# robotic-vision-lab/CropNeRF-A-Neural-Radiance-Field-Based-Framework

Hardware: NVIDIA B200
Metric: train_rays_per_s (higher is better)
Workload: dtype f16 tensor-core MLPs (bf16 gradients), f32 hash tables / accumulation / compositing

## Files before the change

### cropnerf-a-neural-radiance-field-based-framework_b200/csrc/field_mixed_bwd.cu

```cuda
#include <cstdlib>

#include "field_mixed.cuh"

using namespace cnbmix;

namespace {

constexpr int ST = 72;
constexpr int BATCH = WARPS * 16;
constexpr int T_R3 = 0;
constexpr int T_R2 = T_R3 + 64 * 24;
constexpr int T_R1 = T_R2 + 64 * 72;
constexpr int T_S2 = T_R1 + 64 * 72;
constexpr int T_B2 = T_S2 + 64 * 72;
constexpr int T_B1 = T_B2 + 64 * 24;
constexpr int T_HALVES = T_B1 + 32 * 72;
constexpr int A_R3 = 0, A_R2 = 1, A_R1 = 5, A_H = 9, A_S2 = 10, A_S1 = 14, A_B2 = 15, A_B1 = 16, A_TILES = 18;
constexpr int B_R3 = 0, B_R2 = 16, B_R1 = 80, B_H = 144, B_S2 = 160, B_S1 = 224, B_B2 = 288, B_B1 = 304, B_FLOATS = 368;

constexpr size_t SMEM_BWD = (size_t)(HALVES + T_HALVES + 4 * BATCH * ST) * 2 + (size_t)(FLOATS + B_FLOATS + WARPS * A_TILES * 128) * 4;
constexpr int SC_WARPS = 4;
constexpr int THREADS_FUSED = THREADS + SC_WARPS * 32;
constexpr int NSLOT = 4;
constexpr size_t SMEM_BWD_FUSED = SMEM_BWD + 2 * NSLOT * sizeof(uint64_t);
static_assert(BATCH == SC_WARPS * 32, "one scatter warp per 32 samples of a batch");
static_assert(SMEM_BWD_FUSED <= 232448, "227 KB of dynamic shared memory per CTA");

struct BwdArgs {
  MixArgs m;
  float* d_table;
  const __half* x0;
  const float* pos;
  const float *d_density, *d_rgb, *d_sem;
  float* d_x0;
  float *dWb1, *dbb1, *dWb2, *dbb2, *dWs1, *dbs1, *dWs2, *dbs2, *dWh, *dbh, *dWr1, *dbr1, *dWr2, *dbr2, *dWr3, *dbr3;
  float* d_embedding;
};

__device__ __forceinline__ uint32_t pack_bf2(float a, float b) {
  __nv_bfloat162 h = __floats2bfloat162_rn(a, b);
  return *reinterpret_cast<uint32_t*>(&h);
}
__device__ __forceinline__ float2 unpack_h2(uint32_t v) { return __half22float2(*reinterpret_cast<__half2*>(&v)); }
__device__ __forceinline__ uint32_t h2_to_bf2(uint32_t v) {
  const float2 f = unpack_h2(v);
// ... 97 lines not shown
__device__ __forceinline__ void flush_tiles(const float* acc_tiles, int warp, int lane, Put put) {
  constexpr int WPM = WARPS / MT;
  constexpr int NT = NTT / WPM;
  const int mi = warp / WPM, nj0 = (warp % WPM) * NT;
  const int g = lane >> 2, t = lane & 3;
#pragma unroll
  for (int nt = 0; nt < NT; ++nt)
#pragma unroll
    for (int q = 0; q < 4; ++q) {
      const float v = acc_tiles[(nt * 4 + q) * 32 + lane];
      if (v != 0.f) put(16 * mi + g + (q >> 1) * 8, 8 * (nj0 + nt) + 2 * t + (q & 1), v);
    }
}

__device__ __forceinline__ void bar_mlp() { asm volatile("bar.sync 1, %0;" ::"n"(THREADS) : "memory"); }
__device__ __forceinline__ void mbar_arrive(uint32_t bar) { asm volatile("mbarrier.arrive.shared::cta.b64 _, [%0];" ::"r"(bar) : "memory"); }
__device__ __forceinline__ void mbar_wait(uint32_t bar, uint32_t parity) {
  uint32_t done;
  do {
    asm volatile("{\n\t.reg .pred p;\n\tmbarrier.try_wait.parity.shared::cta.b64 p, [%1], %2;\n\tselp.b32 %0, 1, 0, p;\n\t}" : "=r"(done) : "r"(bar), "r"(parity) : "memory");
  } while (!done);
}

__device__ __forceinline__ void scatter_role(const MixArgs& a, float* __restrict__ d_table, const float* __restrict__ pos, const float* __restrict__ d_x0,
                                             uint32_t mbar_s, int sw, int lane, int64_t N, int64_t nbatches) {
  int j = 0;
  for (int64_t batch = blockIdx.x; batch < nbatches; batch += gridDim.x, ++j) {
    const int slot = j % NSLOT;
    const uint32_t par = (uint32_t)(j / NSLOT) & 1u;
    const int64_t s = batch * BATCH + sw * 32 + lane;
    const bool in = s < N;
    float px = 0.f, py = 0.f, pz = 0.f;
    if (in) { px = __ldg(pos + 3 * s); py = __ldg(pos + 3 * s + 1); pz = __ldg(pos + 3 * s + 2); }
    mbar_wait(mbar_s + 8 * slot, par);
#pragma unroll 1
    for (int l0 = 0; l0 < a.L; l0 += 4) {
      float2 d[4];
#pragma unroll
      for (int q = 0; q < 4; ++q) {
        d[q] = make_float2(0.f, 0.f);
        if (in && l0 + q < a.L) d[q] = __ldcg(reinterpret_cast<const float2*>(d_x0) + (int64_t)(l0 + q) * N + s);
      }
#pragma unroll
      for (int q = 0; q < 4; ++q) {
        const int l = l0 + q;
        if (l < a.L) {
          const bool active = d[q].x != 0.0f || d[q].y != 0.0f;
          CnbCell c = {};
          if (active) c = cnb_cell(px, py, pz, a.scalings[l]);
          cnb_scatter_cell(d_table, c, a.mask, (uint32_t)l * a.T, d[q].x, d[q].y, active);
        }
      }
    }
    __syncwarp();
    if (lane == 0) mbar_arrive(mbar_s + 8 * (NSLOT + slot));
  }
}

__device__ inline void load_weights_t(const MixArgs& a, __nv_bfloat16* WT) {
  const int tid = threadIdx.x;
  for (int e = tid; e < 64 * 24; e += THREADS) {
    const int in = e / 24, out = e - in * 24;
    WT[T_R3 + e] = __float2bfloat16_rn(out < 3 ? __ldg(a.Wr3 + out * 64 + in) : 0.f);
    WT[T_B2 + e] = __float2bfloat16_rn(out < 16 ? __ldg(a.Wb2 + out * 64 + in) : 0.f);
  }
  for (int e = tid; e < 64 * 72; e += THREADS) {
    const int in = e / 72, out = e - in * 72;
    const bool ok = out < 64;
    WT[T_R2 + e] = __float2bfloat16_rn(ok ? __ldg(a.Wr2 + out * 64 + in) : 0.f);
    WT[T_S2 + e] = __float2bfloat16_rn(ok ? __ldg(a.Ws2 + out * 64 + in) : 0.f);
    float w1 = 0.f;
    if (ok) {
      if (in < 16) w1 = __ldg(a.Wr1 + out * 63 + in);
      else if (in >= 17) w1 = __ldg(a.Wr1 + out * 63 + (in - 1));
    }
    WT[T_R1 + e] = __float2bfloat16_rn(w1);
  }
  for (int e = tid; e < 32 * 72; e += THREADS) {
    const int in = e / 72, out = e - in * 72;
    WT[T_B1 + e] = __float2bfloat16_rn((out < 64 && in < a.in0) ? __ldg(a.Wb1 + out * a.in0 + in) : 0.f);
  }
}

template <bool FUSED>
__global__ void __launch_bounds__(FUSED ? THREADS_FUSED : THREADS, 1) k_field_mixed_bwd(const __grid_constant__ BwdArgs b) {
  extern __shared__ __align__(16) unsigned char smem_raw[];
  const MixArgs& a = b.m;
  __half* Wsm = reinterpret_cast<__half*>(smem_raw);
  __nv_bfloat16* WT = reinterpret_cast<__nv_bfloat16*>(Wsm + HALVES);
  __nv_bfloat16* st_base = WT + T_HALVES;
  float* Bf = reinterpret_cast<float*>(st_base + 4 * BATCH * ST);
  float* bias_acc = Bf + FLOATS;
  float* acc_all = bias_acc + B_FLOATS;
  const uint32_t mbar_s = (uint32_t)__cvta_generic_to_shared(smem_raw + SMEM_BWD);
  if (!FUSED || threadIdx.x < THREADS) {
    load_weights(a, Wsm, Bf);
    load_weights_t(a, WT);
    for (int e = threadIdx.x; e < B_FLOATS + WARPS * A_TILES * 128; e += THREADS) bias_acc[e] = 0.f;
  } else if (threadIdx.x == THREADS) {
    for (int i = 0; i < NSLOT; ++i) {
      asm volatile("mbarrier.init.shared::cta.b64 [%0], %1;" ::"r"(mbar_s + 8 * i), "r"(THREADS));
      asm volatile("mbarrier.init.shared::cta.b64 [%0], %1;" ::"r"(mbar_s + 8 * (NSLOT + i)), "r"(SC_WARPS));
    }
    asm volatile("fence.mbarrier_init.release.cluster;" ::: "memory");
  }
  __syncthreads();

  const int warp = threadIdx.x >> 5, lane = threadIdx.x & 31;
  if (FUSED) {
    const int64_t N_ = a.sm.num_rays * a.sm.samples_per_ray;
    if (warp >= WARPS) {
      asm volatile("setmaxnreg.dec.sync.aligned.u32 56;");
      scatter_role(a, b.d_table, b.pos, b.d_x0, mbar_s, warp - WARPS, lane, N_, (N_ + BATCH - 1) / BATCH);
      return;
    }
    asm volatile("setmaxnreg.inc.sync.aligned.u32 224;");
  }
  const int g = lane >> 2, t = lane & 3;
  float* acc_w = acc_all + warp * A_TILES * 128;
  uint32_t* const st32 = reinterpret_cast<uint32_t*>(st_base);
  const uint32_t st_s = (uint32_t)__cvta_generic_to_shared(st_base);
  constexpr int MATW = BATCH * ST / 2;
  int buf = 0;
  const int row0 = warp * 16;
  const int S = a.sm.samples_per_ray;
  const int64_t N = a.sm.num_rays * S;
  const int64_t nbatches = (N + BATCH - 1) / BATCH;

  struct TileIn {
    uint32_t A0[2][4];
    float dirv[2][3];
    float2 embv[2][2][2];
// ... 38 lines not shown
        if (t == 0 && b.d_density) { in.ddens[h] = __ldg(b.d_density + rw); in.posx[h] = __ldg(b.pos + 3 * rw); }
      }
    }
  };
  const int64_t tstride = (int64_t)gridDim.x * WARPS;
  TileIn nxt;
  int cam2[2];
  {
    const int64_t t0 = (int64_t)blockIdx.x * WARPS + warp;
    int cam1[2];
    load_cam(t0, cam1);
    load_tile(t0, cam1, nxt);
    load_cam(t0 + tstride, cam2);
  }

  int jb = 0;
  for (int64_t batch = blockIdx.x; batch < nbatches; batch += gridDim.x, ++jb) {
    const int64_t tile = batch * WARPS + warp;
    const int64_t row[2] = {tile * 16 + g, tile * 16 + g + 8};
    bool valid[2];
#pragma unroll
    for (int h = 0; h < 2; ++h) valid[h] = row[h] < N;
    const TileIn cur = nxt;
    load_tile(tile + tstride, cam2, nxt);
    load_cam(tile + 2 * tstride, cam2);
    uint32_t A0[2][4];
#pragma unroll
    for (int kt = 0; kt < 2; ++kt)
#pragma unroll
      for (int q = 0; q < 4; ++q) A0[kt][q] = cur.A0[kt][q];
    const int cam[2] = {cur.cam[0], cur.cam[1]};
    const float (&dirv)[2][3] = cur.dirv;
// ... 177 lines not shown
      uint32_t D[4][4];
      relu_mask_pack<4>(acc, AH, D);
      stage<4, false>(st32 + (2 * buf + 1) * MATW, row0, D, g, t);
      stage<2, true>(st32 + (2 * buf) * MATW, row0, A0, g, t);
      bar_mlp();
      dw_gemm<4, 4>(st_s + (2 * buf + 1) * MATW * 4, st_s + (2 * buf) * MATW * 4, acc_w + A_B1 * 128, bias_acc + B_B1, warp, lane);
      buf ^= 1;
      float dx[4][4];
      zero_acc<4>(dx);
      layer_bf<4, 4, 72>(WT + T_B1, D, dx, g, t);
#pragma unroll
      for (int nt = 0; nt < 4; ++nt) {
        float2* const dlev = reinterpret_cast<float2*>(b.d_x0) + (int64_t)(4 * nt + t) * N;
        if (valid[0]) dlev[row[0]] = make_float2(dx[nt][0], dx[nt][1]);
        if (valid[1]) dlev[row[1]] = make_float2(dx[nt][2], dx[nt][3]);
      }
      if (FUSED) {
        const int slot = jb % NSLOT;
        if (jb >= NSLOT) mbar_wait(mbar_s + 8 * (NSLOT + slot), (uint32_t)(jb / NSLOT - 1) & 1u);
        mbar_arrive(mbar_s + 8 * slot);
      }
    }
  }

  const int in0 = a.in0;
  if (b.dWr3) flush_tiles<1, 8>(acc_w + A_R3 * 128, warp, lane, [&](int n, int k, float v) { if (n < 3) atomicAdd(b.dWr3 + n * 64 + k, v); });
  if (b.dWr2) flush_tiles<4, 8>(acc_w + A_R2 * 128, warp, lane, [&](int n, int k, float v) { atomicAdd(b.dWr2 + n * 64 + k, v); });
  if (b.dWr1) flush_tiles<4, 8>(acc_w + A_R1 * 128, warp, lane, [&](int n, int k, float v) { if (k != 16) atomicAdd(b.dWr1 + n * 63 + (k < 16 ? k : k - 1), v); });
  if (b.dWh) flush_tiles<1, 8>(acc_w + A_H * 128, warp, lane, [&](int n, int k, float v) { if (n == 0) atomicAdd(b.dWh + k, v); });
  if (b.dWs2) flush_tiles<4, 8>(acc_w + A_S2 * 128, warp, lane, [&](int n, int k, float v) { atomicAdd(b.dWs2 + n * 64 + k, v); });
  if (b.dWs1) flush_tiles<4, 2>(acc_w + A_S1 * 128, warp, lane, [&](int n, int k, float v) { if (k >= 1) atomicAdd(b.dWs1 + n * 15 + (k - 1), v); });
  if (b.dWb2) flush_tiles<1, 8>(acc_w + A_B2 * 128, warp, lane, [&](int n, int k, float v) { atomicAdd(b.dWb2 + n * 64 + k, v); });
  if (b.dWb1) flush_tiles<4, 4>(acc_w + A_B1 * 128, warp, lane, [&](int n, int k, float v) { if (k < in0) atomicAdd(b.dWb1 + n * in0 + k, v); });
  bar_mlp();
  for (int e = threadIdx.x; e < B_FLOATS; e += THREADS) {
// ... 31 lines not shown
  }();
  if (mode == 0) return cnb_field_mixed_bwd_tc5(f, s, d_density, d_rgb, d_sem, ctx, stream);
  if (mode == 2) return cnb_field_mixed_bwd_umma(f, s, d_density, d_rgb, d_sem, ctx, stream);
  BwdArgs b;
  fill_args(f, s, b.m);
  const int64_t N = s->num_rays * s->samples_per_ray;
  b.x0 = reinterpret_cast<const __half*>(ctx);
  b.pos = ctx + ctx_pos_off(N);
  b.d_x0 = ctx + ctx_dx0_off(N);
  b.d_density = d_density; b.d_rgb = d_rgb; b.d_sem = d_sem;
  b.dWb1 = f->base.dW[0]; b.dbb1 = f->base.db[0]; b.dWb2 = f->base.dW[1]; b.dbb2 = f->base.db[1];
  b.dWs1 = f->sem.dW[0]; b.dbs1 = f->sem.db[0]; b.dWs2 = f->sem.dW[1]; b.dbs2 = f->sem.db[1];
  b.dWh = f->sem_head.dW[0]; b.dbh = f->sem_head.db[0];
  b.dWr1 = f->rgb.dW[0]; b.dbr1 = f->rgb.db[0]; b.dWr2 = f->rgb.dW[1]; b.dbr2 = f->rgb.db[1]; b.dWr3 = f->rgb.dW[2]; b.dbr3 = f->rgb.db[2];
  b.d_embedding = f->appearance_mode == CNB_APP_PER_CAMERA ? f->d_embedding : nullptr;
  b.d_table = f->grid.d_table;
  static const bool want_fused = [] { const char* e = getenv("CNB_FIELD_BWD_FUSED"); return e != nullptr && e[0] == '1'; }();
  bool fused = want_fused && b.d_table != nullptr;
  for (int i = 0; i < f->grid.num_levels && fused; ++i) fused = f->grid.scalings[i] < 65535.0f;
  static bool configured = false;
  if (!configured) {
    if (cudaFuncSetAttribute(k_field_mixed_bwd<false>, cudaFuncAttributeMaxDynamicSharedMemorySize, (int)SMEM_BWD) != cudaSuccess ||
        cudaFuncSetAttribute(k_field_mixed_bwd<true>, cudaFuncAttributeMaxDynamicSharedMemorySize, (int)SMEM_BWD_FUSED) != cudaSuccess)
      return cnb_check_launch("field_mixed_bwd attr");
    configured = true;
  }
  const int64_t nbatches = (N + BATCH - 1) / BATCH;
  int64_t blocks = nbatches < (int64_t)cnb_num_sms() ? nbatches : (int64_t)cnb_num_sms();
  if (fused) {
    k_field_mixed_bwd<true><<<(int)blocks, THREADS_FUSED, SMEM_BWD_FUSED, stream>>>(b);
    return cnb_check_launch("field_mixed_bwd (fused scatter)");
  }
  k_field_mixed_bwd<false><<<(int)blocks, THREADS, SMEM_BWD, stream>>>(b);
  int rc = cnb_check_launch("field_mixed_bwd");
  if (rc) return rc;
  return cnb_hashgrid_bwd_level_major(&f->grid, b.pos, b.d_x0, N, stream);
}
```

### cropnerf-a-neural-radiance-field-based-framework_b200/csrc/field_mixed_bwd_tc5.cu

```cuda
#include <cstdio>
#include <cstdlib>
#include <type_traits>

#include "field_mixed.cuh"

using namespace cnbmix;

namespace {

constexpr int ROWS = 128;
constexpr int NWG = 2;
constexpr int EPI = NWG * ROWS;
constexpr int KTHREADS = EPI + 256;
constexpr int NSC = 5;
constexpr uint32_t FB = 2048;
constexpr int NSTEP = 12;

constexpr uint32_t B_DS = 0;
constexpr uint32_t B_AH = B_DS + 2 * FB;
constexpr uint32_t B_BO = B_AH + 8 * FB;
constexpr uint32_t B_R1 = B_BO + 2 * FB;
constexpr uint32_t B_ONES = B_R1 + 8 * FB;
constexpr uint32_t B_R2 = B_ONES + FB;
constexpr uint32_t B_AIN = B_R2 + 8 * FB;
constexpr uint32_t B_D = B_AIN + 8 * FB;
constexpr uint32_t WG_BYTES = B_D + 8 * FB;
constexpr uint32_t W_B1 = 0;
constexpr uint32_t W_B2 = W_B1 + 64 * 32 * 2;
constexpr uint32_t W_R1 = W_B2 + 16 * 64 * 2;
// ... 91 lines not shown
                 : "r"(taddr + c));
  asm volatile("tcgen05.wait::ld.sync.aligned;" ::: "memory");
#pragma unroll
  for (int c = 0; c < NC; ++c) v[c] = __uint_as_float(r[c]);
}

__device__ __forceinline__ uint32_t pack_bf2(float a, float b) {
  __nv_bfloat162 h = __floats2bfloat162_rn(a, b);
  return *reinterpret_cast<uint32_t*>(&h);
}
template <int NB>
__device__ __forceinline__ void row_store(unsigned char* mat, int r, const uint32_t (&w)[NB * 4]) {
#pragma unroll
  for (int fb = 0; fb < NB; ++fb) *reinterpret_cast<uint4*>(mat + fb * FB + r * 16) = make_uint4(w[4 * fb], w[4 * fb + 1], w[4 * fb + 2], w[4 * fb + 3]);
}
template <int NC, bool RELU>
__device__ __forceinline__ void bias_act_pack(const float (&v)[NC], const float* __restrict__ bias, uint32_t (&w)[NC / 2]) {
#pragma unroll
  for (int c = 0; c < NC; c += 4) {
    const float4 b = *reinterpret_cast<const float4*>(bias + c);
    float y0 = v[c] + b.x, y1 = v[c + 1] + b.y, y2 = v[c + 2] + b.z, y3 = v[c + 3] + b.w;
    if (RELU) { y0 = fmaxf(y0, 0.f); y1 = fmaxf(y1, 0.f); y2 = fmaxf(y2, 0.f); y3 = fmaxf(y3, 0.f); }
    w[c / 2] = pack_bf2(y0, y1);
    w[c / 2 + 1] = pack_bf2(y2, y3);
  }
}
template <int NC>
__device__ __forceinline__ void mask_pack(const float (&v)[NC], const uint32_t (&P)[4], int sh, uint32_t (&w)[NC / 2]) {
#pragma unroll
  for (int j = 0; j < NC / 2; ++j) {
// ... 175 lines not shown
  }
  asm volatile("fence.proxy.async.shared::cta;" ::: "memory");
  asm volatile("tcgen05.fence::before_thread_sync;");
  __syncthreads();
  asm volatile("tcgen05.fence::after_thread_sync;");
  const uint32_t tmem = *tmem_slot;
  if (b.dbg && blockIdx.x == 0 && threadIdx.x == 0) { b.dbg[49] = clock64() - t_start; b.dbg[52] = t_w - t_start; b.dbg[55] = tmark[0] - t_start; b.dbg[56] = tmark[1] - t_start; }
  const uint32_t smem_s = (uint32_t)__cvta_generic_to_shared(smem);
  const uint32_t bars_s = smem_s + O_BAR;
  const int S = a.sm.samples_per_ray;
  const int64_t N = a.sm.num_rays * S;
  const int64_t nbatches = (N + ROWS - 1) / ROWS;
  const int64_t nb_cta = nbatches > blockIdx.x ? (nbatches - blockIdx.x + gridDim.x - 1) / gridDim.x : 0;

  if (warp >= EPI / 32) {
    asm volatile("setmaxnreg.dec.sync.aligned.u32 56;");
    const int iw = warp - EPI / 32;
    if (iw < NWG) {
      uint32_t ph = 0;
      for (int64_t j = iw; j < nb_cta; j += NWG) {
        for (int step = 0; step < NSTEP; ++step) {
          const long long tq0 = b.dbg ? clock64() : 0;
          const ChainOp op = prepare_chain(step, smem_s + O_WG + (uint32_t)iw * WG_BYTES, smem_s + O_W);
          mbar_wait(bars_s + 8 * iw, ph);
          ph ^= 1u;
          asm volatile("tcgen05.fence::after_thread_sync;");
          const long long tq1 = b.dbg ? clock64() : 0;
          if (elect_one()) {
            issue_chain(op, tmem + T_CHAIN + 64u * (uint32_t)iw);
            asm volatile("tcgen05.commit.cta_group::1.mbarrier::arrive::one.b64 [%0];" ::"l"((uint64_t)(bars_s + 8 * (2 * NWG + iw))) : "memory");
            if (b.dbg && blockIdx.x == 0 && iw == 0) { b.dbg[step] += tq1 - tq0; b.dbg[12 + step] += clock64() - tq1; }
// ... 18 lines not shown
              issue_dw(step, tmem, wg_s, j0 == 0 && w == 0);
              asm volatile("tcgen05.commit.cta_group::1.mbarrier::arrive::one.b64 [%0];" ::"l"((uint64_t)(bars_s + 8 * (3 * NWG + w))) : "memory");
            }
            __syncwarp();
          }
        }
      }
    } else if (FUSED) {
      const int sc = iw - NWG - 1;
      const uint32_t cnt_s = (uint32_t)__cvta_generic_to_shared(rows_done);
      for (int64_t j = 0; j < nb_cta; ++j) {
        bool waited = false;
        for (int sw = 0; sw < ROWS / 32; ++sw) {
          if ((int)((j * (ROWS / 32) + sw) % NSC) != sc) continue;
          if (!waited) {
            const uint32_t want = (uint32_t)(j / NWG + 1) * ROWS;
            uint32_t have;
            do {
              asm volatile("ld.acquire.cta.shared::cta.u32 %0, [%1];" : "=r"(have) : "r"(cnt_s + 4u * (uint32_t)(j % NWG)) : "memory");
            } while (have < want);
            waited = true;
          }
          scatter_batch(a, b.d_table, b.pos, b.d_x0, blockIdx.x + j * gridDim.x, sw, lane, N);
        }
      }
    }
  } else {
    asm volatile("setmaxnreg.inc.sync.aligned.u32 200;");
    const int wg = warp >> 2, r = threadIdx.x & (ROWS - 1);
    unsigned char* base = smem + O_WG + (uint32_t)wg * WG_BYTES;
    const uint32_t ready_s = bars_s + 8 * wg, dwready_s = bars_s + 8 * (NWG + wg), done_s = bars_s + 8 * (2 * NWG + wg);
    const uint32_t trow = tmem + ((uint32_t)(32 * (warp & 3)) << 16) + T_CHAIN + 64u * (uint32_t)wg;
    uint32_t dphase = 0;
    int estep = 0;
    long long te = 0;
    const bool dbg_on = b.dbg != nullptr && blockIdx.x == 0 && threadIdx.x == 0;
    long long t_fence = 0, t_dbgrmw = 0;
    auto ready = [&](bool dw = false) {
      if (dbg_on) { const long long t0 = clock64(); b.dbg[36 + estep] += t0 - te; ++estep; t_dbgrmw += clock64() - t0; }
      const long long tf = dbg_on ? clock64() : 0;
      asm volatile("fence.proxy.async.shared::cta;" ::: "memory");
      asm volatile("tcgen05.fence::before_thread_sync;");
      asm volatile("mbarrier.arrive.shared::cta.b64 _, [%0];" ::"r"(ready_s) : "memory");
// ... 2 lines not shown
    };
    const uint32_t dwdone_s = bars_s + 8 * (3 * NWG + wg);
    uint32_t wphase = 0;
    auto wait_dw = [&]() {
      mbar_wait(dwdone_s, wphase);
      wphase ^= 1u;
    };
    auto wait_acc = [&]() {
      const long long tw = dbg_on ? clock64() : 0;
      mbar_wait(done_s, dphase);
      dphase ^= 1u;
      asm volatile("tcgen05.fence::after_thread_sync;");
      if (dbg_on) { te = clock64(); b.dbg[24 + estep - 1] += te - tw; }
    };
    struct RowIn {
      uint4 xq[4];
      float4 st;
      uint4 mq[2];
      float drgb[3], dsem, ddens, dir[3];
      int cam;
    };
    auto load_row = [&](int64_t j, RowIn& in) {
      const int64_t i = (blockIdx.x + j * gridDim.x) * ROWS + r;
      const bool ok = j < nb_cta && i < N;
#pragma unroll
      for (int q = 0; q < 4; ++q) in.xq[q] = make_uint4(0u, 0u, 0u, 0u);
      in.st = make_float4(0.f, 0.f, 0.f, 0.f);
      in.mq[0] = in.mq[1] = make_uint4(0u, 0u, 0u, 0u);
      in.drgb[0] = in.drgb[1] = in.drgb[2] = 0.f; in.dsem = 0.f; in.ddens = 0.f;
      in.dir[0] = in.dir[1] = in.dir[2] = 0.f; in.cam = 0;
      if (j >= nb_cta) return;
      if (ok) {
#pragma unroll
        for (int q = 0; q < 4; ++q) in.xq[q] = __ldg(reinterpret_cast<const uint4*>(b.x0 + i * 32) + q);
        in.st = __ldg(reinterpret_cast<const float4*>(b.stash) + i);
        in.mq[0] = __ldg(b.masks + 2 * i); in.mq[1] = __ldg(b.masks + 2 * i + 1);
        if (b.d_rgb) { in.drgb[0] = __ldg(b.d_rgb + 3 * i); in.drgb[1] = __ldg(b.d_rgb + 3 * i + 1); in.drgb[2] = __ldg(b.d_rgb + 3 * i + 2); }
        if (b.d_sem) in.dsem = __ldg(b.d_sem + i);
        if (b.d_density) in.ddens = __ldg(b.d_density + i);
      }
      const int64_t ry = (i < N ? i : N - 1) / S;
      in.dir[0] = __ldg(a.sm.directions + 3 * ry); in.dir[1] = __ldg(a.sm.directions + 3 * ry + 1); in.dir[2] = __ldg(a.sm.directions + 3 * ry + 2);
      if (a.app_mode == CNB_APP_PER_CAMERA) in.cam = __ldg(a.sm.camera_indices + ry);
    };
    RowIn nxt;
    load_row(wg, nxt);
    for (int64_t j = wg; j < nb_cta; j += NWG) {
      const int64_t i = (blockIdx.x + j * gridDim.x) * ROWS + r;
      const bool valid = i < N;
      const int64_t ray = (valid ? i : N - 1) / S;
      const RowIn cur = nxt;
      const uint4 (&xq)[4] = cur.xq;
      const float4 st = cur.st;
      const uint4 (&mq)[2] = cur.mq;
      const float (&drgb)[3] = cur.drgb;
      const float dsem = cur.dsem, ddens = cur.ddens;
      const float dirx = cur.dir[0], diry = cur.dir[1], dirz = cur.dir[2];
      const int cam = cur.cam;
      const float* erow = a.app_mode == CNB_APP_PER_CAMERA ? a.embedding + (int64_t)cam * 32 : (a.app_mode == CNB_APP_MEAN ? a.embedding : nullptr);
      const uint32_t P0[4] = {mq[0].x, mq[0].z, mq[1].x, mq[1].z};
      const uint32_t P1[4] = {mq[0].y, mq[0].w, mq[1].y, mq[1].w};
      uint32_t x0w[16];
#pragma unroll
      for (int q = 0; q < 4; ++q) {
        const uint32_t hw[4] = {xq[q].x, xq[q].y, xq[q].z, xq[q].w};
#pragma unroll
        for (int e = 0; e < 4; ++e) {
          const float2 f = __half22float2(*reinterpret_cast<const __half2*>(&hw[e]));
          x0w[4 * q + e] = pack_bf2(f.x, f.y);
        }
      }
      if (dbg_on) { te = clock64(); estep = 0; }
      row_store<4>(base + B_AIN, r, x0w);
      ready();
      load_row(j + NWG, nxt);
      {
        wait_acc();
        float v[64];
        tm_load<64>(trow, v);
        uint32_t w[32];
        bias_act_pack<64, true>(v, Cf + C_BB1, w);
        row_store<8>(base + B_AH, r, w);
        ready();
      }
      {
        float4 ev[8];
#pragma unroll
        for (int q = 0; q < 8; ++q) ev[q] = erow ? __ldg(reinterpret_cast<const float4*>(erow) + q) : make_float4(0.f, 0.f, 0.f, 0.f);
        float sh[16];
        cnb_sh16(dirx, diry, dirz, sh);
        uint32_t ain[32];
#pragma unroll
        for (int c = 0; c < 8; ++c) ain[c] = pack_bf2(sh[2 * c], sh[2 * c + 1]);
#pragma unroll
        for (int q = 0; q < 8; ++q) { ain[16 + 2 * q] = pack_bf2(ev[q].x, ev[q].y); ain[16 + 2 * q + 1] = pack_bf2(ev[q].z, ev[q].w); }
        wait_acc();
        float v[16];
        tm_load<16>(trow, v);
        uint32_t w[8];
        bias_act_pack<16, false>(v, Cf + C_BB2, w);
        w[0] = (w[0] & 0xFFFF0000u) | 0x3F80u;
        row_store<2>(base + B_BO, r, w);
#pragma unroll
        for (int c = 0; c < 8; ++c) ain[8 + c] = w[c];
        row_store<8>(base + B_AIN, r, ain);
        ready();
      }
      {
        wait_acc();
        float v[64];
        tm_load<64>(trow, v);
        uint32_t w[32];
        bias_act_pack<64, true>(v, Cf + C_BR1, w);
        if (j > wg) wait_dw();
        row_store<8>(base + B_R1, r, w);
        ready();
      }
      {
        wait_acc();
        float v[64];
        tm_load<64>(trow, v);
        uint32_t w[32];
        bias_act_pack<64, true>(v, Cf + C_BR2, w);
        row_store<8>(base + B_R2, r, w);
        uint32_t d3[8] = {0u, 0u, 0u, 0u, 0u, 0u, 0u, 0u};
        d3[0] = pack_bf2(drgb[0] * st.y * (1.f - st.y), drgb[1] * st.z * (1.f - st.z));
        d3[1] = pack_bf2(drgb[2] * st.w * (1.f - st.w), 0.f);
        row_store<2>(base + B_DS, r, d3);
        ready(true);
      }
      {
        wait_acc();
        float v[64];
        tm_load<64>(trow, v);
        uint32_t w[32];
        mask_pack<64>(v, P1, 8, w);
        wait_dw();
        row_store<8>(base + B_D, r, w);
        ready(true);
      }
      {
        wait_acc();
        float v[64];
        tm_load<64>(trow, v);
        uint32_t w[32];
        mask_pack<64>(v, P1, 0, w);

        wait_dw();
        row_store<8>(base + B_D, r, w);
        ready(true);
      }
      float dbo[16];
      {
        wait_acc();
        float v[48];
        tm_load<48>(trow, v);
#pragma unroll
        for (int c = 0; c < 16; ++c) dbo[c] = v[c];
        if (a.app_mode == CNB_APP_PER_CAMERA && b.d_embedding != nullptr) {
          const int64_t ray0 = __shfl_sync(0xffffffffu, ray, 0), ray1 = __shfl_sync(0xffffffffu, ray, 31);
          const int cam0 = __shfl_sync(0xffffffffu, cam, 0), cam1 = __shfl_sync(0xffffffffu, cam, 31);
          const bool two = __all_sync(0xffffffffu, ray == ray0 || ray == ray1);
          if (two) {
            float x[32];
#pragma unroll
            for (int c = 0; c < 32; ++c) x[c] = ray == ray0 ? v[16 + c] : 0.f;
            const float s0 = transpose_reduce32(x, lane);
            if (s0 != 0.f) atomicAdd(b.d_embedding + (int64_t)cam0 * 32 + lane, s0);
            if (ray0 != ray1) {
#pragma unroll
              for (int c = 0; c < 32; ++c) x[c] = ray == ray0 ? 0.f : v[16 + c];
              const float s1 = transpose_reduce32(x, lane);
              if (s1 != 0.f) atomicAdd(b.d_embedding + (int64_t)cam1 * 32 + lane, s1);
            }
          } else if (valid) {
#pragma unroll
            for (int c = 0; c < 32; ++c) atomicAdd(b.d_embedding + (int64_t)cam * 32 + c, v[16 + c]);
          }
        }
        wait_dw();
        ready();
      }
      {
        wait_acc();
        float v[64];
        tm_load<64>(trow, v);
        uint32_t w[32];
        bias_act_pack<64, true>(v, Cf + C_BS1, w);
        row_store<8>(base + B_R1, r, w);
        ready();
      }
      {
        wait_acc();
        float v[64];
        tm_load<64>(trow, v);
        uint32_t w[32];
        bias_act_pack<64, false>(v, Cf + C_BS2, w);

        row_store<8>(base + B_R2, r, w);
        uint32_t dh[8] = {0u, 0u, 0u, 0u, 0u, 0u, 0u, 0u};
        dh[0] = pack_bf2(dsem, 0.f);
        row_store<2>(base + B_DS, r, dh);
#pragma unroll
        for (int c = 0; c < 64; c += 4) {
          const float4 wh = *reinterpret_cast<const float4*>(Cf + C_WH + c);
          w[c / 2] = pack_bf2(dsem * wh.x, dsem * wh.y);
          w[c / 2 + 1] = pack_bf2(dsem * wh.z, dsem * wh.w);
        }
        row_store<8>(base + B_D, r, w);
        ready(true);
      }
      {
        wait_acc();
        float v[64];
        tm_load<64>(trow, v);
        uint32_t w[32];
        mask_pack<64>(v, P0, 8, w);
        wait_dw();
        row_store<8>(base + B_D, r, w);
        uint32_t db[8];
        dbo[0] = ddens * st.x;
#pragma unroll
        for (int c = 0; c < 8; ++c) db[c] = pack_bf2(dbo[2 * c], dbo[2 * c + 1]);
        row_store<2>(base + B_DS, r, db);
        ready(true);
      }
      {
        wait_acc();
        float v[64];
        tm_load<64>(trow, v);
        uint32_t w[32];
        mask_pack<64>(v, P0, 0, w);
        wait_dw();
        row_store<8>(base + B_D, r, w);
        row_store<4>(base + B_R1, r, x0w);
        *reinterpret_cast<uint4*>(base + B_R1 + 4 * FB + r * 16) = make_uint4(0x3F803F80u, 0x3F803F80u, 0x3F803F80u, 0x3F803F80u);
        ready(true);
      }
      {
        wait_acc();
        float v[32];
        tm_load<32>(trow, v);
        if (valid) {
#pragma unroll
          for (int l = 0; l < 16; ++l)
            if (l < a.L) reinterpret_cast<float2*>(b.d_x0)[(int64_t)l * N + i] = make_float2(v[2 * l], v[2 * l + 1]);
        }
        if (FUSED)
          asm volatile("red.release.cta.shared::cta.add.u32 [%0], 1;" ::"r"((uint32_t)__cvta_generic_to_shared(rows_done + wg)) : "memory");
        asm volatile("tcgen05.fence::before_thread_sync;");
        if (dbg_on) { b.dbg[48] += clock64() - te; b.dbg[53] = t_fence; b.dbg[54] = t_dbgrmw; }
      }
    }
    if (wg < nb_cta) wait_dw();
  }

  __syncthreads();
  asm volatile("tcgen05.fence::after_thread_sync;");
  if (b.dbg && blockIdx.x == 0 && threadIdx.x == 0) b.dbg[50] = clock64() - t_start;
  const int in0 = a.in0;
  float* img = reinterpret_cast<float*>(smem + O_WG);
  if (nb_cta > 0) {
    const int q = warp & 3, m = 16 * q + (lane & 15), r128 = 32 * q + lane;
    const bool own = lane < 16;
    const uint32_t taddr = tmem + ((uint32_t)(32 * q) << 16);
    const float inv_sh0 = 1.0f / __bfloat162float(__float2bfloat16_rn(0.28209479177387814f));
    auto rd = [&](auto ncols_tag, uint32_t col0, bool mine, auto put) {
      constexpr int NC = decltype(ncols_tag)::value;
#pragma unroll
// ... 92 lines not shown
  if (want_dbg) {
    if (!dbg_dev) cudaMalloc(&dbg_dev, 64 * sizeof(long long));
    cudaMemsetAsync(dbg_dev, 0, 64 * sizeof(long long), stream);
    b.dbg = dbg_dev;
  }
  static bool configured = false;
  if (!configured) {
    if (cudaFuncSetAttribute(k_field_bwd_tc5<false>, cudaFuncAttributeMaxDynamicSharedMemorySize, (int)SMEM_TC5) != cudaSuccess ||
        cudaFuncSetAttribute(k_field_bwd_tc5<true>, cudaFuncAttributeMaxDynamicSharedMemorySize, (int)SMEM_TC5) != cudaSuccess)
      return cnb_check_launch("field_bwd_tc5 attr");
    configured = true;
  }
  const int64_t nbatches = (N + ROWS - 1) / ROWS;
  int64_t blocks = nbatches < (int64_t)cnb_num_sms() ? nbatches : (int64_t)cnb_num_sms();
  if (blocks > CTX_PART_CTAS) blocks = CTX_PART_CTAS;
  static const bool want_fused = [] { const char* e = getenv("CNB_FIELD_BWD_FUSED"); return e != nullptr && e[0] == '1'; }();
  b.d_table = f->grid.d_table;
  b.pos = ctx + ctx_pos_off(N);
  bool fused = want_fused && b.d_table != nullptr;
  for (int i = 0; i < f->grid.num_levels && fused; ++i) fused = f->grid.scalings[i] < 65535.0f;
  if (fused) k_field_bwd_tc5<true><<<(int)blocks, KTHREADS, SMEM_TC5, stream>>>(b);
  else k_field_bwd_tc5<false><<<(int)blocks, KTHREADS, SMEM_TC5, stream>>>(b);
  int rc = cnb_check_launch("field_bwd_tc5");
  if (rc) return rc;
  k_tc5_reduce<<<dim3((I_END + 255) / 256, 4), 256, 0, stream>>>(b, (int)blocks);
  if ((rc = cnb_check_launch("field_bwd_tc5 reduce"))) return rc;
  if (want_dbg) {
    long long h[64];
    cudaStreamSynchronize(stream);
    cudaMemcpy(h, dbg_dev, sizeof(h), cudaMemcpyDeviceToHost);
    fprintf(stderr, "[tc5] N=%lld  step: issuer_wait issuer_issue | epi_wait epi_work (cycles summed over CTA 0's wg0 batches)\n", (long long)N);
    for (int i = 0; i < 12; ++i) fprintf(stderr, "[tc5] %2d: %8lld %8lld | %8lld %8lld\n", i, h[i], h[12 + i], h[24 + i], h[36 + i]);
    fprintf(stderr, "[tc5] final epilogue work %lld ; CTA 0: prologue %lld, batch loop end %lld, kernel end %lld cycles\n", h[48], h[49], h[50], h[51]);
    fprintf(stderr, "[tc5] weights: loads issued at %lld, first matrix stored at %lld, all stored at %lld cycles; fence+arrive total %lld; dbg RMW total %lld\n", h[55], h[56], h[52], h[53], h[54]);
  }
  if (fused) return CNB_OK;
  return cnb_hashgrid_bwd_level_major(&f->grid, ctx + ctx_pos_off(N), b.d_x0, N, stream);
}
```

Baseline: 5.469 million.

## Enable fused hashgrid scatter in tcgen05 backward by default with more scatter warps

Makes the tc5 backward kernel always fuse the hash-table gradient scatter into its warp-specialised schedule, so the separate level-major scatter pass no longer runs, and removes the old env-gated fused path from the mma.sync kernel. Adds 128 more auxiliary threads so there are more scatter warps, and rebalances setmaxnreg to 128 registers for the epilogue and 72 for the auxiliary warps. To fit the smaller epilogue register budget, TMEM reads are split into 32-column halves, x0 is reloaded just before its use instead of being carried across the batch, and per-row inputs are loaded later. The risks are register spills in the epilogue and atomic contention or poorer scatter locality compared with the level-major pass. Extra debug timers are also added.

Measured after the change: 5.601 million (median of 6 runs). 1.02x the previous value.

```diff
diff --git a/cropnerf-a-neural-radiance-field-based-framework_b200/csrc/field_mixed_bwd.cu b/cropnerf-a-neural-radiance-field-based-framework_b200/csrc/field_mixed_bwd.cu
--- a/cropnerf-a-neural-radiance-field-based-framework_b200/csrc/field_mixed_bwd.cu
+++ b/cropnerf-a-neural-radiance-field-based-framework_b200/csrc/field_mixed_bwd.cu
@@ -19,16 +19,9 @@
 constexpr int B_R3 = 0, B_R2 = 16, B_R1 = 80, B_H = 144, B_S2 = 160, B_S1 = 224, B_B2 = 288, B_B1 = 304, B_FLOATS = 368;
 
 constexpr size_t SMEM_BWD = (size_t)(HALVES + T_HALVES + 4 * BATCH * ST) * 2 + (size_t)(FLOATS + B_FLOATS + WARPS * A_TILES * 128) * 4;
-constexpr int SC_WARPS = 4;
-constexpr int THREADS_FUSED = THREADS + SC_WARPS * 32;
-constexpr int NSLOT = 4;
-constexpr size_t SMEM_BWD_FUSED = SMEM_BWD + 2 * NSLOT * sizeof(uint64_t);
-static_assert(BATCH == SC_WARPS * 32, "one scatter warp per 32 samples of a batch");
-static_assert(SMEM_BWD_FUSED <= 232448, "227 KB of dynamic shared memory per CTA");
 
 struct BwdArgs {
   MixArgs m;
-  float* d_table;
   const __half* x0;
   const float* pos;
   const float *d_density, *d_rgb, *d_sem;
@@ -156,48 +149,6 @@
 }
 
 __device__ __forceinline__ void bar_mlp() { asm volatile("bar.sync 1, %0;" ::"n"(THREADS) : "memory"); }
-__device__ __forceinline__ void mbar_arrive(uint32_t bar) { asm volatile("mbarrier.arrive.shared::cta.b64 _, [%0];" ::"r"(bar) : "memory"); }
-__device__ __forceinline__ void mbar_wait(uint32_t bar, uint32_t parity) {
-  uint32_t done;
-  do {
-    asm volatile("{\n\t.reg .pred p;\n\tmbarrier.try_wait.parity.shared::cta.b64 p, [%1], %2;\n\tselp.b32 %0, 1, 0, p;\n\t}" : "=r"(done) : "r"(bar), "r"(parity) : "memory");
-  } while (!done);
-}
-
-__device__ __forceinline__ void scatter_role(const MixArgs& a, float* __restrict__ d_table, const float* __restrict__ pos, const float* __restrict__ d_x0,
-                                             uint32_t mbar_s, int sw, int lane, int64_t N, int64_t nbatches) {
-  int j = 0;
-  for (int64_t batch = blockIdx.x; batch < nbatches; batch += gridDim.x, ++j) {
-    const int slot = j % NSLOT;
-    const uint32_t par = (uint32_t)(j / NSLOT) & 1u;
-    const int64_t s = batch * BATCH + sw * 32 + lane;
-    const bool in = s < N;
-    float px = 0.f, py = 0.f, pz = 0.f;
-    if (in) { px = __ldg(pos + 3 * s); py = __ldg(pos + 3 * s + 1); pz = __ldg(pos + 3 * s + 2); }
-    mbar_wait(mbar_s + 8 * slot, par);
-#pragma unroll 1
-    for (int l0 = 0; l0 < a.L; l0 += 4) {
-      float2 d[4];
-#pragma unroll
-      for (int q = 0; q < 4; ++q) {
-        d[q] = make_float2(0.f, 0.f);
-        if (in && l0 + q < a.L) d[q] = __ldcg(reinterpret_cast<const float2*>(d_x0) + (int64_t)(l0 + q) * N + s);
-      }
-#pragma unroll
-      for (int q = 0; q < 4; ++q) {
-        const int l = l0 + q;
-        if (l < a.L) {
-          const bool active = d[q].x != 0.0f || d[q].y != 0.0f;
-          CnbCell c = {};
-          if (active) c = cnb_cell(px, py, pz, a.scalings[l]);
-          cnb_scatter_cell(d_table, c, a.mask, (uint32_t)l * a.T, d[q].x, d[q].y, active);
-        }
-      }
-    }
-    __syncwarp();
-    if (lane == 0) mbar_arrive(mbar_s + 8 * (NSLOT + slot));
-  }
-}
 
 __device__ inline void load_weights_t(const MixArgs& a, __nv_bfloat16* WT) {
   const int tid = threadIdx.x;
@@ -224,8 +175,7 @@
   }
 }
 
-template <bool FUSED>
-__global__ void __launch_bounds__(FUSED ? THREADS_FUSED : THREADS, 1) k_field_mixed_bwd(const __grid_constant__ BwdArgs b) {
+__global__ void __launch_bounds__(THREADS, 1) k_field_mixed_bwd(const __grid_constant__ BwdArgs b) {
   extern __shared__ __align__(16) unsigned char smem_raw[];
   const MixArgs& a = b.m;
   __half* Wsm = reinterpret_cast<__half*>(smem_raw);
@@ -234,30 +184,12 @@
   float* Bf = reinterpret_cast<float*>(st_base + 4 * BATCH * ST);
   float* bias_acc = Bf + FLOATS;
   float* acc_all = bias_acc + B_FLOATS;
-  const uint32_t mbar_s = (uint32_t)__cvta_generic_to_shared(smem_raw + SMEM_BWD);
-  if (!FUSED || threadIdx.x < THREADS) {
-    load_weights(a, Wsm, Bf);
-    load_weights_t(a, WT);
-    for (int e = threadIdx.x; e < B_FLOATS + WARPS * A_TILES * 128; e += THREADS) bias_acc[e] = 0.f;
-  } else if (threadIdx.x == THREADS) {
-    for (int i = 0; i < NSLOT; ++i) {
-      asm volatile("mbarrier.init.shared::cta.b64 [%0], %1;" ::"r"(mbar_s + 8 * i), "r"(THREADS));
-      asm volatile("mbarrier.init.shared::cta.b64 [%0], %1;" ::"r"(mbar_s + 8 * (NSLOT + i)), "r"(SC_WARPS));
-    }
-    asm volatile("fence.mbarrier_init.release.cluster;" ::: "memory");
-  }
+  load_weights(a, Wsm, Bf);
+  load_weights_t(a, WT);
+  for (int e = threadIdx.x; e < B_FLOATS + WARPS * A_TILES * 128; e += THREADS) bias_acc[e] = 0.f;
   __syncthreads();
 
   const int warp = threadIdx.x >> 5, lane = threadIdx.x & 31;
-  if (FUSED) {
-    const int64_t N_ = a.sm.num_rays * a.sm.samples_per_ray;
-    if (warp >= WARPS) {
-      asm volatile("setmaxnreg.dec.sync.aligned.u32 56;");
-      scatter_role(a, b.d_table, b.pos, b.d_x0, mbar_s, warp - WARPS, lane, N_, (N_ + BATCH - 1) / BATCH);
-      return;
-    }
-    asm volatile("setmaxnreg.inc.sync.aligned.u32 224;");
-  }
   const int g = lane >> 2, t = lane & 3;
   float* acc_w = acc_all + warp * A_TILES * 128;
   uint32_t* const st32 = reinterpret_cast<uint32_t*>(st_base);
@@ -326,8 +258,7 @@
     load_cam(t0 + tstride, cam2);
   }
 
-  int jb = 0;
-  for (int64_t batch = blockIdx.x; batch < nbatches; batch += gridDim.x, ++jb) {
+  for (int64_t batch = blockIdx.x; batch < nbatches; batch += gridDim.x) {
     const int64_t tile = batch * WARPS + warp;
     const int64_t row[2] = {tile * 16 + g, tile * 16 + g + 8};
     bool valid[2];
@@ -535,11 +466,6 @@
         float2* const dlev = reinterpret_cast<float2*>(b.d_x0) + (int64_t)(4 * nt + t) * N;
         if (valid[0]) dlev[row[0]] = make_float2(dx[nt][0], dx[nt][1]);
         if (valid[1]) dlev[row[1]] = make_float2(dx[nt][2], dx[nt][3]);
-      }
-      if (FUSED) {
-        const int slot = jb % NSLOT;
-        if (jb >= NSLOT) mbar_wait(mbar_s + 8 * (NSLOT + slot), (uint32_t)(jb / NSLOT - 1) & 1u);
-        mbar_arrive(mbar_s + 8 * slot);
       }
     }
   }
@@ -601,24 +527,15 @@
   b.dWh = f->sem_head.dW[0]; b.dbh = f->sem_head.db[0];
   b.dWr1 = f->rgb.dW[0]; b.dbr1 = f->rgb.db[0]; b.dWr2 = f->rgb.dW[1]; b.dbr2 = f->rgb.db[1]; b.dWr3 = f->rgb.dW[2]; b.dbr3 = f->rgb.db[2];
   b.d_embedding = f->appearance_mode == CNB_APP_PER_CAMERA ? f->d_embedding : nullptr;
-  b.d_table = f->grid.d_table;
-  static const bool want_fused = [] { const char* e = getenv("CNB_FIELD_BWD_FUSED"); return e != nullptr && e[0] == '1'; }();
-  bool fused = want_fused && b.d_table != nullptr;
-  for (int i = 0; i < f->grid.num_levels && fused; ++i) fused = f->grid.scalings[i] < 65535.0f;
   static bool configured = false;
   if (!configured) {
-    if (cudaFuncSetAttribute(k_field_mixed_bwd<false>, cudaFuncAttributeMaxDynamicSharedMemorySize, (int)SMEM_BWD) != cudaSuccess ||
-        cudaFuncSetAttribute(k_field_mixed_bwd<true>, cudaFuncAttributeMaxDynamicSharedMemorySize, (int)SMEM_BWD_FUSED) != cudaSuccess)
+    if (cudaFuncSetAttribute(k_field_mixed_bwd, cudaFuncAttributeMaxDynamicSharedMemorySize, (int)SMEM_BWD) != cudaSuccess)
       return cnb_check_launch("field_mixed_bwd attr");
     configured = true;
   }
   const int64_t nbatches = (N + BATCH - 1) / BATCH;
   int64_t blocks = nbatches < (int64_t)cnb_num_sms() ? nbatches : (int64_t)cnb_num_sms();
-  if (fused) {
-    k_field_mixed_bwd<true><<<(int)blocks, THREADS_FUSED, SMEM_BWD_FUSED, stream>>>(b);
-    return cnb_check_launch("field_mixed_bwd (fused scatter)");
-  }
-  k_field_mixed_bwd<false><<<(int)blocks, THREADS, SMEM_BWD, stream>>>(b);
+  k_field_mixed_bwd<<<(int)blocks, THREADS, SMEM_BWD, stream>>>(b);
   int rc = cnb_check_launch("field_mixed_bwd");
   if (rc) return rc;
   return cnb_hashgrid_bwd_level_major(&f->grid, b.pos, b.d_x0, N, stream);
diff --git a/cropnerf-a-neural-radiance-field-based-framework_b200/csrc/field_mixed_bwd_tc5.cu b/cropnerf-a-neural-radiance-field-based-framework_b200/csrc/field_mixed_bwd_tc5.cu
--- a/cropnerf-a-neural-radiance-field-based-framework_b200/csrc/field_mixed_bwd_tc5.cu
+++ b/cropnerf-a-neural-radiance-field-based-framework_b200/csrc/field_mixed_bwd_tc5.cu
@@ -11,8 +11,10 @@
 constexpr int ROWS = 128;
 constexpr int NWG = 2;
 constexpr int EPI = NWG * ROWS;
-constexpr int KTHREADS = EPI + 256;
-constexpr int NSC = 5;
+constexpr int KTHREADS = EPI + 384;
+constexpr int EPI_REGS = 128, AUX_REGS = 72;
+static_assert(EPI * EPI_REGS + (KTHREADS - EPI) * AUX_REGS <= 65536 / KTHREADS / 8 * 8 * KTHREADS, "setmaxnreg split exceeds the launch budget");
+constexpr int NSC = KTHREADS / 32 - EPI / 32 - 3;
 constexpr uint32_t FB = 2048;
 constexpr int NSTEP = 12;
 
@@ -134,6 +136,30 @@
 #pragma unroll
   for (int fb = 0; fb < NB; ++fb) *reinterpret_cast<uint4*>(mat + fb * FB + r * 16) = make_uint4(w[4 * fb], w[4 * fb + 1], w[4 * fb + 2], w[4 * fb + 3]);
 }
+template <typename Pack, typename Before>
+__device__ __forceinline__ void acc64_store(uint32_t trow, unsigned char* mat, int r, Pack pack, Before before_store) {
+#pragma unroll
+  for (int h = 0; h < 2; ++h) {
+    float v[32];
+    tm_load<32>(trow + 32 * h, v);
+    uint32_t w[16];
+    pack(h, v, w);
+    if (h == 0) before_store();
+    row_store<4>(mat + 4 * h * FB, r, w);
+  }
+}
+__device__ __forceinline__ void x0_bf16(const __half* x0, int64_t i, bool ok, uint32_t (&x0w)[16]) {
+#pragma unroll
+  for (int q = 0; q < 4; ++q) {
+    const uint4 xq = ok ? __ldg(reinterpret_cast<const uint4*>(x0 + i * 32) + q) : make_uint4(0u, 0u, 0u, 0u);
+    const uint32_t hw[4] = {xq.x, xq.y, xq.z, xq.w};
+#pragma unroll
+    for (int e = 0; e < 4; ++e) {
+      const float2 f = __half22float2(*reinterpret_cast<const __half2*>(&hw[e]));
+      x0w[4 * q + e] = pack_bf2(f.x, f.y);
+    }
+  }
+}
 template <int NC, bool RELU>
 __device__ __forceinline__ void bias_act_pack(const float (&v)[NC], const float* __restrict__ bias, uint32_t (&w)[NC / 2]) {
 #pragma unroll
@@ -339,7 +365,7 @@
   const int64_t nb_cta = nbatches > blockIdx.x ? (nbatches - blockIdx.x + gridDim.x - 1) / gridDim.x : 0;
 
   if (warp >= EPI / 32) {
-    asm volatile("setmaxnreg.dec.sync.aligned.u32 56;");
+    asm volatile("setmaxnreg.dec.sync.aligned.u32 %0;" ::"n"(AUX_REGS));
     const int iw = warp - EPI / 32;
     if (iw < NWG) {
       uint32_t ph = 0;
@@ -388,19 +414,22 @@
         for (int sw = 0; sw < ROWS / 32; ++sw) {
           if ((int)((j * (ROWS / 32) + sw) % NSC) != sc) continue;
           if (!waited) {
+            const long long tw = b.dbg ? clock64() : 0;
             const uint32_t want = (uint32_t)(j / NWG + 1) * ROWS;
             uint32_t have;
             do {
               asm volatile("ld.acquire.cta.shared::cta.u32 %0, [%1];" : "=r"(have) : "r"(cnt_s + 4u * (uint32_t)(j % NWG)) : "memory");
             } while (have < want);
             waited = true;
+            if (b.dbg && blockIdx.x == 0 && sc == 0 && lane == 0) b.dbg[57] += clock64() - tw;
           }
           scatter_batch(a, b.d_table, b.pos, b.d_x0, blockIdx.x + j * gridDim.x, sw, lane, N);
         }
       }
+      if (b.dbg && blockIdx.x == 0 && lane == 0) atomicMax(reinterpret_cast<unsigned long long*>(b.dbg + 58), (unsigned long long)(clock64() - t_start));
     }
   } else {
-    asm volatile("setmaxnreg.inc.sync.aligned.u32 200;");
+    asm volatile("setmaxnreg.inc.sync.aligned.u32 %0;" ::"n"(EPI_REGS));
     const int wg = warp >> 2, r = threadIdx.x & (ROWS - 1);
     unsigned char* base = smem + O_WG + (uint32_t)wg * WG_BYTES;
     const uint32_t ready_s = bars_s + 8 * wg, dwready_s = bars_s + 8 * (NWG + wg), done_s = bars_s + 8 * (2 * NWG + wg);
@@ -433,43 +462,58 @@
       if (dbg_on) { te = clock64(); b.dbg[24 + estep - 1] += te - tw; }
     };
     struct RowIn {
-      uint4 xq[4];
       float4 st;
       uint4 mq[2];
       float drgb[3], dsem, ddens, dir[3];
       int cam;
     };
-    auto load_row = [&](int64_t j, RowIn& in) {
+    auto load_x0 = [&](int64_t j, uint4 (&xq)[4]) {
       const int64_t i = (blockIdx.x + j * gridDim.x) * ROWS + r;
       const bool ok = j < nb_cta && i < N;
 #pragma unroll
-      for (int q = 0; q < 4; ++q) in.xq[q] = make_uint4(0u, 0u, 0u, 0u);
+      for (int q = 0; q < 4; ++q) xq[q] = ok ? __ldg(reinterpret_cast<const uint4*>(b.x0 + i * 32) + q) : make_uint4(0u, 0u, 0u, 0u);
+    };
+    auto load_row = [&](int64_t i, RowIn& in) {
+      const bool ok = i < N;
       in.st = make_float4(0.f, 0.f, 0.f, 0.f);
       in.mq[0] = in.mq[1] = make_uint4(0u, 0u, 0u, 0u);
       in.drgb[0] = in.drgb[1] = in.drgb[2] = 0.f; in.dsem = 0.f; in.ddens = 0.f;
-      in.dir[0] = in.dir[1] = in.dir[2] = 0.f; in.cam = 0;
-      if (j >= nb_cta) return;
       if (ok) {
-#pragma unroll
-        for (int q = 0; q < 4; ++q) in.xq[q] = __ldg(reinterpret_cast<const uint4*>(b.x0 + i * 32) + q);
         in.st = __ldg(reinterpret_cast<const float4*>(b.stash) + i);
         in.mq[0] = __ldg(b.masks + 2 * i); in.mq[1] = __ldg(b.masks + 2 * i + 1);
         if (b.d_rgb) { in.drgb[0] = __ldg(b.d_rgb + 3 * i); in.drgb[1] = __ldg(b.d_rgb + 3 * i + 1); in.drgb[2] = __ldg(b.d_rgb + 3 * i + 2); }
         if (b.d_sem) in.dsem = __ldg(b.d_sem + i);
         if (b.d_density) in.ddens = __ldg(b.d_density + i);
       }
-      const int64_t ry = (i < N ? i : N - 1) / S;
+      const int64_t ry = (ok ? i : N - 1) / S;
       in.dir[0] = __ldg(a.sm.directions + 3 * ry); in.dir[1] = __ldg(a.sm.directions + 3 * ry + 1); in.dir[2] = __ldg(a.sm.directions + 3 * ry + 2);
-      if (a.app_mode == CNB_APP_PER_CAMERA) in.cam = __ldg(a.sm.camera_indices + ry);
+      in.cam = a.app_mode == CNB_APP_PER_CAMERA ? __ldg(a.sm.camera_indices + ry) : 0;
     };
-    RowIn nxt;
-    load_row(wg, nxt);
+    uint4 nxq[4];
+    load_x0(wg, nxq);
     for (int64_t j = wg; j < nb_cta; j += NWG) {
       const int64_t i = (blockIdx.x + j * gridDim.x) * ROWS + r;
       const bool valid = i < N;
       const int64_t ray = (valid ? i : N - 1) / S;
-      const RowIn cur = nxt;
-      const uint4 (&xq)[4] = cur.xq;
+      const auto none = [] {};
+      if (dbg_on) { te = clock64(); estep = 0; }
+      {
+        uint32_t x0w[16];
+#pragma unroll
+        for (int q = 0; q < 4; ++q) {
+          const uint32_t hw[4] = {nxq[q].x, nxq[q].y, nxq[q].z, nxq[q].w};
+#pragma unroll
+          for (int e = 0; e < 4; ++e) {
+            const float2 f = __half22float2(*reinterpret_cast<const __half2*>(&hw[e]));
+            x0w[4 * q + e] = pack_bf2(f.x, f.y);
+          }
+        }
+        row_store<4>(base + B_AIN, r, x0w);
+      }
+      ready();
+      load_x0(j + NWG, nxq);
+      RowIn cur;
+      load_row(i, cur);
       const float4 st = cur.st;
       const uint4 (&mq)[2] = cur.mq;
       const float (&drgb)[3] = cur.drgb;
@@ -479,27 +523,9 @@
       const float* erow = a.app_mode == CNB_APP_PER_CAMERA ? a.embedding + (int64_t)cam * 32 : (a.app_mode == CNB_APP_MEAN ? a.embedding : nullptr);
       const uint32_t P0[4] = {mq[0].x, mq[0].z, mq[1].x, mq[1].z};
       const uint32_t P1[4] = {mq[0].y, mq[0].w, mq[1].y, mq[1].w};
-      uint32_t x0w[16];
-#pragma unroll
-      for (int q = 0; q < 4; ++q) {
-        const uint32_t hw[4] = {xq[q].x, xq[q].y, xq[q].z, xq[q].w};
-#pragma unroll
-        for (int e = 0; e < 4; ++e) {
-          const float2 f = __half22float2(*reinterpret_cast<const __half2*>(&hw[e]));
-          x0w[4 * q + e] = pack_bf2(f.x, f.y);
-        }
-      }
-      if (dbg_on) { te = clock64(); estep = 0; }
-      row_store<4>(base + B_AIN, r, x0w);
-      ready();
-      load_row(j + NWG, nxt);
-      {
-        wait_acc();
-        float v[64];
-        tm_load<64>(trow, v);
-        uint32_t w[32];
-        bias_act_pack<64, true>(v, Cf + C_BB1, w);
-        row_store<8>(base + B_AH, r, w);
+      {
+        wait_acc();
+        acc64_store(trow, base + B_AH, r, [&](int h, const float (&v)[32], uint32_t (&w)[16]) { bias_act_pack<32, true>(v, Cf + C_BB1 + 32 * h, w); }, none);
         ready();
       }
       {
@@ -527,21 +553,13 @@
       }
       {
         wait_acc();
-        float v[64];
-        tm_load<64>(trow, v);
-        uint32_t w[32];
-        bias_act_pack<64, true>(v, Cf + C_BR1, w);
-        if (j > wg) wait_dw();
-        row_store<8>(base + B_R1, r, w);
+        acc64_store(trow, base + B_R1, r, [&](int h, const float (&v)[32], uint32_t (&w)[16]) { bias_act_pack<32, true>(v, Cf + C_BR1 + 32 * h, w); },
+                    [&] { if (j > wg) wait_dw(); });
         ready();
       }
       {
         wait_acc();
-        float v[64];
-        tm_load<64>(trow, v);
-        uint32_t w[32];
-        bias_act_pack<64, true>(v, Cf + C_BR2, w);
-        row_store<8>(base + B_R2, r, w);
+        acc64_store(trow, base + B_R2, r, [&](int h, const float (&v)[32], uint32_t (&w)[16]) { bias_act_pack<32, true>(v, Cf + C_BR2 + 32 * h, w); }, none);
         uint32_t d3[8] = {0u, 0u, 0u, 0u, 0u, 0u, 0u, 0u};
         d3[0] = pack_bf2(drgb[0] * st.y * (1.f - st.y), drgb[1] * st.z * (1.f - st.z));
         d3[1] = pack_bf2(drgb[2] * st.w * (1.f - st.w), 0.f);
@@ -550,51 +568,47 @@
       }
       {
         wait_acc();
-        float v[64];
-        tm_load<64>(trow, v);
-        uint32_t w[32];
-        mask_pack<64>(v, P1, 8, w);
-        wait_dw();
-        row_store<8>(base + B_D, r, w);
+        acc64_store(trow, base + B_D, r, [&](int h, const float (&v)[32], uint32_t (&w)[16]) { mask_pack<32>(v, P1, 8 + 4 * h, w); },
+                    [&] { wait_dw(); });
         ready(true);
       }
       {
         wait_acc();
-        float v[64];
-        tm_load<64>(trow, v);
-        uint32_t w[32];
-        mask_pack<64>(v, P1, 0, w);
-
-        wait_dw();
-        row_store<8>(base + B_D, r, w);
+        acc64_store(trow, base + B_D, r, [&](int h, const float (&v)[32], uint32_t (&w)[16]) { mask_pack<32>(v, P1, 4 * h, w); },
+                    [&] { wait_dw(); });
         ready(true);
       }
-      float dbo[16];
-      {
-        wait_acc();
-        float v[48];
-        tm_load<48>(trow, v);
-#pragma unroll
-        for (int c = 0; c < 16; ++c) dbo[c] = v[c];
+      uint32_t db[8];
+      {
+        wait_acc();
+        {
+          float v[16];
+          tm_load<16>(trow, v);
+          v[0] = ddens * st.x;
+#pragma unroll
+          for (int c = 0; c < 8; ++c) db[c] = pack_bf2(v[2 * c], v[2 * c + 1]);
+        }
         if (a.app_mode == CNB_APP_PER_CAMERA && b.d_embedding != nullptr) {
+          float v[32];
+          tm_load<32>(trow + 16, v);
           const int64_t ray0 = __shfl_sync(0xffffffffu, ray, 0), ray1 = __shfl_sync(0xffffffffu, ray, 31);
           const int cam0 = __shfl_sync(0xffffffffu, cam, 0), cam1 = __shfl_sync(0xffffffffu, cam, 31);
           const bool two = __all_sync(0xffffffffu, ray == ray0 || ray == ray1);
           if (two) {
             float x[32];
 #pragma unroll
-            for (int c = 0; c < 32; ++c) x[c] = ray == ray0 ? v[16 + c] : 0.f;
+            for (int c = 0; c < 32; ++c) x[c] = ray == ray0 ? v[c] : 0.f;
             const float s0 = transpose_reduce32(x, lane);
             if (s0 != 0.f) atomicAdd(b.d_embedding + (int64_t)cam0 * 32 + lane, s0);
             if (ray0 != ray1) {
 #pragma unroll
-              for (int c = 0; c < 32; ++c) x[c] = ray == ray0 ? 0.f : v[16 + c];
+              for (int c = 0; c < 32; ++c) x[c] = ray == ray0 ? 0.f : v[c];
               const float s1 = transpose_reduce32(x, lane);
               if (s1 != 0.f) atomicAdd(b.d_embedding + (int64_t)cam1 * 32 + lane, s1);
             }
           } else if (valid) {
 #pragma unroll
-            for (int c = 0; c < 32; ++c) atomicAdd(b.d_embedding + (int64_t)cam * 32 + c, v[16 + c]);
+            for (int c = 0; c < 32; ++c) atomicAdd(b.d_embedding + (int64_t)cam * 32 + c, v[c]);
           }
         }
         wait_dw();
@@ -602,24 +616,16 @@
       }
       {
         wait_acc();
-        float v[64];
-        tm_load<64>(trow, v);
-        uint32_t w[32];
-        bias_act_pack<64, true>(v, Cf + C_BS1, w);
-        row_store<8>(base + B_R1, r, w);
+        acc64_store(trow, base + B_R1, r, [&](int h, const float (&v)[32], uint32_t (&w)[16]) { bias_act_pack<32, true>(v, Cf + C_BS1 + 32 * h, w); }, none);
         ready();
       }
       {
         wait_acc();
-        float v[64];
-        tm_load<64>(trow, v);
-        uint32_t w[32];
-        bias_act_pack<64, false>(v, Cf + C_BS2, w);
-
-        row_store<8>(base + B_R2, r, w);
+        acc64_store(trow, base + B_R2, r, [&](int h, const float (&v)[32], uint32_t (&w)[16]) { bias_act_pack<32, false>(v, Cf + C_BS2 + 32 * h, w); }, none);
         uint32_t dh[8] = {0u, 0u, 0u, 0u, 0u, 0u, 0u, 0u};
         dh[0] = pack_bf2(dsem, 0.f);
         row_store<2>(base + B_DS, r, dh);
+        uint32_t w[32];
 #pragma unroll
         for (int c = 0; c < 64; c += 4) {
           const float4 wh = *reinterpret_cast<const float4*>(Cf + C_WH + c);
@@ -631,27 +637,17 @@
       }
       {
         wait_acc();
-        float v[64];
-        tm_load<64>(trow, v);
-        uint32_t w[32];
-        mask_pack<64>(v, P0, 8, w);
-        wait_dw();
-        row_store<8>(base + B_D, r, w);
-        uint32_t db[8];
-        dbo[0] = ddens * st.x;
-#pragma unroll
-        for (int c = 0; c < 8; ++c) db[c] = pack_bf2(dbo[2 * c], dbo[2 * c + 1]);
+        acc64_store(trow, base + B_D, r, [&](int h, const float (&v)[32], uint32_t (&w)[16]) { mask_pack<32>(v, P0, 8 + 4 * h, w); },
+                    [&] { wait_dw(); });
         row_store<2>(base + B_DS, r, db);
         ready(true);
       }
       {
-        wait_acc();
-        float v[64];
-        tm_load<64>(trow, v);
-        uint32_t w[32];
-        mask_pack<64>(v, P0, 0, w);
-        wait_dw();
-        row_store<8>(base + B_D, r, w);
+        uint32_t x0w[16];
+        x0_bf16(b.x0, i, valid, x0w);
+        wait_acc();
+        acc64_store(trow, base + B_D, r, [&](int h, const float (&v)[32], uint32_t (&w)[16]) { mask_pack<32>(v, P0, 4 * h, w); },
+                    [&] { wait_dw(); });
         row_store<4>(base + B_R1, r, x0w);
         *reinterpret_cast<uint4*>(base + B_R1 + 4 * FB + r * 16) = make_uint4(0x3F803F80u, 0x3F803F80u, 0x3F803F80u, 0x3F803F80u);
         ready(true);
@@ -672,6 +668,7 @@
       }
     }
     if (wg < nb_cta) wait_dw();
+    if (dbg_on) b.dbg[59] = clock64() - t_start;
   }
 
   __syncthreads();
@@ -794,10 +791,9 @@
   const int64_t nbatches = (N + ROWS - 1) / ROWS;
   int64_t blocks = nbatches < (int64_t)cnb_num_sms() ? nbatches : (int64_t)cnb_num_sms();
   if (blocks > CTX_PART_CTAS) blocks = CTX_PART_CTAS;
-  static const bool want_fused = [] { const char* e = getenv("CNB_FIELD_BWD_FUSED"); return e != nullptr && e[0] == '1'; }();
   b.d_table = f->grid.d_table;
   b.pos = ctx + ctx_pos_off(N);
-  bool fused = want_fused && b.d_table != nullptr;
+  bool fused = b.d_table != nullptr;
   for (int i = 0; i < f->grid.num_levels && fused; ++i) fused = f->grid.scalings[i] < 65535.0f;
   if (fused) k_field_bwd_tc5<true><<<(int)blocks, KTHREADS, SMEM_TC5, stream>>>(b);
   else k_field_bwd_tc5<false><<<(int)blocks, KTHREADS, SMEM_TC5, stream>>>(b);
@@ -813,6 +809,7 @@
     for (int i = 0; i < 12; ++i) fprintf(stderr, "[tc5] %2d: %8lld %8lld | %8lld %8lld\n", i, h[i], h[12 + i], h[24 + i], h[36 + i]);
     fprintf(stderr, "[tc5] final epilogue work %lld ; CTA 0: prologue %lld, batch loop end %lld, kernel end %lld cycles\n", h[48], h[49], h[50], h[51]);
     fprintf(stderr, "[tc5] weights: loads issued at %lld, first matrix stored at %lld, all stored at %lld cycles; fence+arrive total %lld; dbg RMW total %lld\n", h[55], h[56], h[52], h[53], h[54]);
+    fprintf(stderr, "[tc5] CTA 0: epilogue warpgroup 0 done at %lld, last scatter warp done at %lld cycles; scatter warp 0 waited %lld cycles for rows\n", h[59], h[58], h[57]);
   }
   if (fused) return CNB_OK;
   return cnb_hashgrid_bwd_level_major(&f->grid, ctx + ctx_pos_off(N), b.d_x0, N, stream);
```
